# wizyoung/YOLOv3_TensorFlow

Measured on AMD Instinct MI355X. Metric: images/sec at 416x416 bs=32 (Darknet-53 + 3-scale head forward), higher is better.
Workload: dtype f32

## Files before the change

include/yolo355.h:

```cpp
#ifndef YOLO355_H
#define YOLO355_H

#include <stddef.h>
#include <stdint.h>

#ifdef __cplusplus
extern "C" {
#endif

#define Y3_OK 0
#define Y3_EINVAL (-1)
#define Y3_EHIP (-2)
#define Y3_ESTATE (-3)

#define Y3_ABI_VERSION 5

typedef struct y3_ctx y3_ctx;
typedef struct y3_net y3_net;
typedef struct y3_train_var y3_train_var;

const char* y3_last_error(void);
int y3_abi_version(void);

int y3_ctx_create(int device, void* stream, y3_ctx** out);
// ... 15 lines not shown
    int stride;
    int act;
} y3_conv_desc;

size_t y3_conv_workspace_bytes(const y3_conv_desc* d);
int y3_streamk_range(int kind, int units, int ksteps, int workers, int group, int local_worker, long long* begin,
                     long long* end);
int y3_conv_image_ranges(const y3_conv_desc* d, int dz_stride, long long limit, int max_ranges, int* begin, int* count);
void y3_debug_conv_range_limit(long long elements);
int y3_conv2d_fwd(y3_ctx* ctx, const y3_conv_desc* d, const float* x, const float* x_up,
                  const float* w, const float* scale, const float* shift, const float* residual,
                  float* y, void* workspace, size_t workspace_bytes);

int y3_conv2d_fwd_stem_s2(y3_ctx* ctx, int n, int h, int w, const float* x, const float* w0_hwio, const float* scale0,
                          const float* shift0, const float* w1_packed, const float* scale1, const float* shift1, float* y);

int y3_pack_conv_weights_bf16(y3_ctx* ctx, const float* w_hwio, int k, int cin, int cout, void* w_packed);
int y3_conv_bf16_tile(const y3_conv_desc* d);
int y3_conv2d_fwd_bf16(y3_ctx* ctx, const y3_conv_desc* d, const void* x, const void* x_up, const void* w,
                       const float* scale, const float* shift, const void* residual, void* y, int out_f32);

int y3_conv2d_fwd_bf16_stem_s2(y3_ctx* ctx, int n, int h, int w, const float* x, const float* w0_hwio, const float* scale0,
                               const float* shift0, const void* w1_packed, const float* scale1, const float* shift1, void* y);

int y3_resblock64_fwd_bf16(y3_ctx* ctx, int n, int h, int w, const void* x, const void* w2_packed, const float* scale2,
                           const float* shift2, const void* w3_packed, const float* scale3, const float* shift3, void* y);

int y3_conv_wino_eligible(const y3_conv_desc* d);
int y3_pack_conv_weights_wino(y3_ctx* ctx, const float* w_hwio, int cin, int cout, float* w_wino);
size_t y3_conv_wino_workspace_bytes(const y3_conv_desc* d);
// ... 40 lines not shown

int y3_net_create(y3_ctx* ctx, int class_num, y3_net** out);
int y3_net_destroy(y3_net* net);
int y3_net_set_dtype(y3_net* net, int dtype);
int y3_net_num_layers(const y3_net* net);
int y3_net_layer_info(const y3_net* net, int i, int* k, int* stride, int* cin, int* cout, int* has_bn);
size_t y3_net_params_bytes(const y3_net* net);
int y3_net_set_params(y3_net* net, const y3_train_var* vars, void* params, size_t params_bytes);
size_t y3_net_workspace_bytes(const y3_net* net, int n, int h, int w);
int y3_net_forward(y3_net* net, const float* x, int n, int h, int w, void* workspace,
                   size_t workspace_bytes, float* fm1, float* fm2, float* fm3);
int y3_net_set_profiling(y3_net* net, int enabled);
int y3_net_get_layer_ms(y3_net* net, float* ms, int count);
int y3_net_layer_is_streamk(const y3_net* net, int i, int n, int h, int w);
int y3_net_layer_fused(const y3_net* net, int i, int n, int h, int w);

int y3_net_layer_graph(const y3_net* net, int i, int* src, int* up, int* resid, int* dst, int* act);
int y3_net_num_tensors(const y3_net* net);
int y3_net_tensor_info(const y3_net* net, int t, int* channels, int* sdiv, int* ext);


size_t y3_reduce_scratch_bytes(int c);
int y3_bn_train_stats(y3_ctx* ctx, const float* z, long long rows, int c, const float* gamma, const float* beta,
                      float eps, float decay, float* mean, float* inv_std, float* scale, float* shift,
                      float* moving_mean, float* moving_var, float* scratch);
int y3_conv_stats_blocks(const y3_conv_desc* d, int wino);
int y3_conv2d_fwd_stats(y3_ctx* ctx, const y3_conv_desc* d, const float* x, const float* w, const float* scale,
                        const float* shift, float* y, float* stats, void* workspace, size_t workspace_bytes);
int y3_conv2d_fwd_wino_stats(y3_ctx* ctx, const y3_conv_desc* d, const float* x, const float* w_wino, const float* scale,
                             const float* shift, float* y, float* stats, void* workspace, size_t workspace_bytes);
// ... 197 lines not shown
```

yolov3_tensorflow_amd/_lib.py:

```python
import ctypes
import os
from ctypes import POINTER, c_char_p, c_double, c_float, c_int, c_longlong, c_size_t, c_void_p

HERE = os.path.dirname(os.path.abspath(__file__))
LIB_PATH = os.environ.get("Y3_LIB_PATH") or os.path.join(HERE, "csrc", "libyolo355.so")

Y3_OK, Y3_EINVAL, Y3_EHIP, Y3_ESTATE = 0, -1, -2, -3
Y3_NMS_TF, Y3_NMS_PY = 0, 1


class ConvDesc(ctypes.Structure):
    _fields_ = [(n, c_int) for n in ("n", "h", "w", "cin", "c_up", "cout", "k", "stride", "act")]


class ParamDesc(ctypes.Structure):
    _fields_ = [("w", c_void_p), ("g", c_void_p), ("slot0", c_void_p), ("slot1", c_void_p), ("n", c_longlong),
                ("weight_decay", c_float), ("reserved", c_int)]


class TrainVar(ctypes.Structure):
    _fields_ = [("weights", c_void_p), ("gamma", c_void_p), ("beta", c_void_p), ("moving_mean", c_void_p),
                ("moving_variance", c_void_p), ("biases", c_void_p), ("g_weights", c_longlong), ("g_gamma", c_longlong),
                ("g_beta", c_longlong), ("g_biases", c_longlong), ("g_end", c_longlong)]

# ... 42 lines not shown
                                   c_void_p, c_void_p, c_size_t]),
    "y3_pack_conv_weights_split": (c_int, [c_void_p, c_void_p, c_int, c_int, c_int, c_int, c_void_p]),
    "y3_conv2d_fwd_split": (c_int, [c_void_p, POINTER(ConvDesc), c_int, c_void_p, c_void_p, c_void_p, c_void_p,
                                    c_void_p, c_void_p, c_void_p, c_void_p, c_size_t]),
    "y3_pack_conv_weights_split_dgrad": (c_int, [c_void_p, c_void_p, c_int, c_int, c_int, c_int, c_void_p]),
    "y3_conv2d_dgrad_split": (c_int, [c_void_p, POINTER(ConvDesc), c_int, c_void_p, c_int, c_void_p, c_void_p, c_void_p,
                                      c_int, c_void_p, c_void_p, c_size_t]),
    "y3_pack_conv_weights_bf16": (c_int, [c_void_p, c_void_p, c_int, c_int, c_int, c_void_p]),
    "y3_conv_bf16_tile": (c_int, [POINTER(ConvDesc)]),
    "y3_conv2d_fwd_bf16": (c_int, [c_void_p, POINTER(ConvDesc), c_void_p, c_void_p, c_void_p, c_void_p, c_void_p,
                                   c_void_p, c_void_p, c_int]),
    "y3_conv2d_fwd_bf16_stem_s2": (c_int, [c_void_p, c_int, c_int, c_int, c_void_p, c_void_p, c_void_p, c_void_p, c_void_p,
                                           c_void_p, c_void_p, c_void_p]),
    "y3_conv2d_fwd_stem_s2": (c_int, [c_void_p, c_int, c_int, c_int, c_void_p, c_void_p, c_void_p, c_void_p, c_void_p,
                                      c_void_p, c_void_p, c_void_p]),
    "y3_resblock64_fwd_bf16": (c_int, [c_void_p, c_int, c_int, c_int, c_void_p, c_void_p, c_void_p, c_void_p, c_void_p,
                                       c_void_p, c_void_p, c_void_p]),
    "y3_net_train_workspace_bytes": (c_size_t, [c_void_p, POINTER(TrainVar), c_int, c_int, c_int]),
    "y3_net_train_forward": (c_int, [c_void_p, POINTER(TrainVar), c_void_p, c_int, c_int, c_int, POINTER(TrainOpts),
                                     c_void_p, c_size_t, POINTER(c_void_p), POINTER(c_void_p), POINTER(c_void_p)]),
    "y3_net_train_loss": (c_int, [c_void_p, c_void_p, c_void_p, c_void_p, POINTER(TrainOpts), c_void_p]),
    "y3_net_train_backward": (c_int, [c_void_p, POINTER(TrainVar), c_void_p, GradReadyFn, c_void_p]),
    "y3_net_train_step": (c_int, [c_void_p, POINTER(TrainVar), c_void_p, c_int, c_int, c_int, c_void_p, c_void_p, c_void_p,
                                  POINTER(TrainOpts), c_void_p, c_void_p, c_size_t, c_void_p, GradReadyFn, c_void_p]),
    "y3_net_train_set_wgrad_stream": (c_int, [c_void_p, c_void_p]),
    "y3_net_train_set_box_loss": (c_int, [c_void_p, c_int]),
    "y3_net_train_set_bn_sync": (c_int, [c_void_p, BnSyncFn, c_void_p, c_void_p, c_size_t]),
    "y3_net_train_saved": (c_int, [c_void_p, c_int, POINTER(c_size_t), POINTER(c_size_t)]),
    "y3_net_train_saved_type": (c_int, [c_void_p, c_int]),
    "y3_pack_conv_weights_bf16_train": (c_int, [c_void_p, c_void_p, c_int, c_int, c_int, c_int, c_void_p]),
# ... 158 lines not shown
```

yolov3_tensorflow_amd/csrc/y3_abi.hip:

```cpp
#include <cstdarg>
#include <cstdio>
#include <cstring>
#include <vector>
#include <algorithm>
#include "y3_internal.h"
#include "y3_net.h"

static thread_local char g_err[512] = "";

void y3_set_error(const char* fmt, ...) {
    va_list ap;
    va_start(ap, fmt);
    vsnprintf(g_err, sizeof(g_err), fmt, ap);
    va_end(ap);
}

extern "C" const char* y3_last_error(void) { return g_err; }

int y3_current_device() {
    int dev = -1;
    if (hipGetDevice(&dev) != hipSuccess || dev < 0 || dev >= Y3_MAX_DEVICES) return -1;
    return dev;
}

// ... 364 lines not shown

extern "C" int y3_net_set_dtype(y3_net* net, int dtype) {
    Y3_CHECK_ARG(net, "y3_net_set_dtype: null net");
    Y3_CHECK_ARG(dtype >= 0 && dtype <= 4,
                 "y3_net_set_dtype: dtype must be 0 (fp32), 1 (bf16), 2 (fp32 via bf16x6), 3 (fp32 via bf16x3) or "
                 "4 (fp32, Winograd for the eligible 3x3 convs)");
    net->dtype = static_cast<NetDtype>(dtype);
    net->pn = net->ph = net->pw = 0;
    for (Layer& l : net->layers) {
        l.scale = l.shift = nullptr;
        std::fill(std::begin(l.w), std::end(l.w), nullptr);
    }
    return Y3_OK;
}

extern "C" int y3_net_destroy(y3_net* net) {
    if (net) {
        for (auto& set : net->event_sets)
            for (hipEvent_t e : set) (void)hipEventDestroy(e);
        if (net->train) y3_train_state_free(net->train);
        if (net->own_stream) (void)hipStreamDestroy(static_cast<hipStream_t>(net->own_stream));
        delete net;
    }
    return Y3_OK;
}

extern "C" int y3_net_num_layers(const y3_net* net) { return net ? (int)net->layers.size() : 0; }

extern "C" int y3_net_layer_info(const y3_net* net, int i, int* k, int* stride, int* cin, int* cout,
                                 int* has_bn) {
// ... 43 lines not shown

static bool fuses_with_next(const y3_net& net, int j, int n, int h, int w) {
    const NetDtype dt = net.dtype;
    const Layer &a = net.layers[j], &b = net.layers[j + 1];
    const Tensor &mid = net.tensors[a.dst], &out = net.tensors[b.dst];
    const y3_conv_desc da = net.desc(j, n, h, w), db = net.desc(j + 1, n, h, w);
    const bool pair = b.src == a.dst && mid.last_use == j + 1 && mid.ext < 0 && out.ext < 0 && a.resid < 0;
    if (j == 0)
        return pair && a.src == 0 && b.resid < 0 &&
               (dt == NetDtype::BF16 ? y3_conv_bf16_stem_s2_takes(&da, &db)
                : (dt == NetDtype::F32 || dt == NetDtype::F32_WINO) && y3_conv_f32_stem_s2_takes(&da, &db)) == 1;
    return j == 2 && dt == NetDtype::BF16 && pair && b.resid == a.src && a.src != 0 && net.tensors[a.src].ext < 0 &&
           y3_conv_bf16_resblock64_takes(&da, &db) == 1;
}

static int split_planes(NetDtype dt) { return dt == NetDtype::F32_BF16X6 ? 3 : dt == NetDtype::F32_BF16X3 ? 2 : 0; }

static ConvRoute fp32_route(const y3_conv_desc& d, bool wino44, bool wino, int planes) {
    ConvRoute r;
    r.kind = wino44 ? RouteKind::Wino44 : wino ? RouteKind::Wino : planes ? RouteKind::Split : RouteKind::Direct;
    r.planes = planes;
    r.two_pass = wino44 && y3_conv_wino44_two_pass_impl(&d);
    r.streamk = !wino44 && !wino && y3_conv_schedule_impl(&d);
    r.scratch = wino44 ? (r.two_pass ? y3_conv_wino44_workspace_bytes_impl(&d) : 0)
                : wino ? y3_conv_wino_workspace_bytes_impl(&d) : y3_conv_workspace_bytes_impl(&d);
    return r;
}

ConvRoute y3_route_infer(const y3_net& net, int i, int n, int h, int w) {
    ConvRoute r;
    const NetDtype dt = net.dtype;
    const y3_conv_desc d = net.desc(i, n, h, w);
    if ((i == 0 || i == 2) && fuses_with_next(net, i, n, h, w)) r.kind = RouteKind::InNext;
    else if ((i == 1 || i == 3) && fuses_with_next(net, i - 1, n, h, w))
        r.kind = i == 3 ? RouteKind::ResBlock64Bf16 : dt == NetDtype::BF16 ? RouteKind::StemS2Bf16 : RouteKind::StemS2F32;
    else if (dt == NetDtype::BF16) r.kind = RouteKind::Bf16;
    else
        r = fp32_route(d, dt == NetDtype::F32_WINO && y3_conv_wino44_preferred_impl(&d),
                       dt == NetDtype::F32_WINO && y3_conv_wino_eligible_impl(&d), split_planes(dt));
    return r;
}

static bool bf16_train(const y3_net& net, int i) { return net.dtype == NetDtype::BF16 && net.layers[i].cin != 3; }

ConvRoute y3_route_train_fwd(const y3_net& net, int i, int n, int h, int w) {
    const Layer& l = net.layers[i];
    const y3_conv_desc d = net.desc(i, n, h, w, true);
    if (bf16_train(net, i)) {
        ConvRoute r;
        r.kind = RouteKind::Bf16Train;
// ... 44 lines not shown
    return r;
}

ConvPack y3_conv_pack(const y3_net& net, int i, const ConvRoute& r, bool dgrad) {
    const Layer& l = net.layers[i];
    ConvPack p;
    p.planes = r.planes; p.dgrad = dgrad;
    p.k = l.k; p.cin = l.cin; p.cout = dgrad ? net.dz_stride(i) : l.cout;
    p.wcout = l.cout;
    switch (r.kind) {
    case RouteKind::Wino44: p.kind = Packing::Wino44; break;
    case RouteKind::Wino: p.kind = Packing::Wino; break;
    case RouteKind::Split: p.kind = Packing::Split; break;
    case RouteKind::Bf16: case RouteKind::StemS2Bf16: case RouteKind::ResBlock64Bf16: p.kind = Packing::Bf16; break;
    case RouteKind::InNext: p.kind = net.dtype == NetDtype::BF16 ? Packing::Bf16 : Packing::Direct; break;
    case RouteKind::Direct: case RouteKind::StemS2F32: p.kind = dgrad ? Packing::Hwio : Packing::Direct; break;
    case RouteKind::Bf16Train: p.kind = Packing::Bf16Reg; break;
    }
    if (l.cin == 3 && !dgrad) p.kind = Packing::Hwio;
    return p;
}

size_t ConvPack::bytes() const {
    const size_t taps = (size_t)k * k * cin * cout;
    switch (kind) {
    case Packing::Direct: return taps * 4;
    case Packing::Bf16: case Packing::Bf16Reg: return taps * 2;
    case Packing::Split: return taps * 2 * planes;
    case Packing::Wino: return (size_t)16 * cin * cout * 4;
    case Packing::Wino44: return (size_t)36 * cin * cout * 4;
    default: return 0;
// ... 90 lines not shown
        }
    }
    for (size_t i = 0; i < net->layers.size(); ++i) {
        Layer& l = net->layers[i];
        l.scale = reinterpret_cast<const float*>(base + lp[i].scale);
        l.shift = reinterpret_cast<const float*>(base + lp[i].shift);
        std::fill(std::begin(l.w), std::end(l.w), nullptr);
        for (size_t j = 0; j < lp[i].packs.size(); ++j) l.w[(int)lp[i].packs[j].kind] = base + lp[i].at[j];
    }
    return Y3_OK;
}

extern "C" int y3_net_layer_fused(const y3_net* net, int i, int n, int h, int w) {
    if (!net || i < 0 || i >= (int)net->layers.size() || n <= 0 || h <= 0 || w <= 0) return 0;
    const RouteKind k = y3_route_infer(*net, i, n, h, w).kind;
    return k == RouteKind::InNext ? 1 : k >= RouteKind::StemS2F32 ? 2 : 0;
}

extern "C" int y3_net_forward(y3_net* net, const float* x, int n, int h, int w, void* workspace,
                              size_t workspace_bytes, float* fm1, float* fm2, float* fm3) {
    Y3_CHECK_ARG(net && x && workspace && fm1 && fm2 && fm3, "y3_net_forward: null argument");
    if (!net->ctx) {
        y3_set_error("y3_net_forward: the net was created without a context");
        return Y3_ESTATE;
    }
    if (int rc = ctx_pending_error(net->ctx)) return rc;
    if (int rc = check_size("y3_net_forward", n, h, w)) return rc;
    net->plan(n, h, w);
    Y3_CHECK_ARG(workspace_bytes >= net->plan_bytes, "y3_net_forward: workspace too small (%zu < %zu)",
                 workspace_bytes, net->plan_bytes);
    Y3_CHECK_ARG(((uintptr_t)workspace & 255) == 0, "y3_net_forward: workspace must be 256-byte aligned");
// ... 30 lines not shown
    if (net->flags_bytes) Y3_CHECK_HIP(hipMemsetAsync(flag_base, 0, net->flags_bytes, st));
    void* scratch = base + net->arena_bytes; const size_t sb = net->scratch_bytes;
    for (size_t i = 0; i < nl; ++i) {
        const Layer& l = net->layers[i];
        const ConvRoute& r = net->routes[i];
        const y3_conv_desc d = net->desc((int)i, n, h, w);
        y3_sk_opts o;
        o.err = net->ctx->err_host;
        o.flags = net->flags_bytes ? flag_base + i * y3_net::FLAG_WORDS : nullptr;
        o.wino44_form = r.two_pass;
        const Layer& p = net->layers[i ? i - 1 : 0];
        const float *pw = wk[i ? i - 1 : 0], *lw = wk[i];
        float *src = ptr(l.src), *up = ptr(l.up), *res = ptr(l.resid), *y = ptr(l.dst);
        int rc = Y3_OK;
        switch (r.kind) {
        case RouteKind::InNext: break;
        case RouteKind::StemS2F32:
            rc = y3_launch_conv_f32_stem_s2(st, n, h, w, x, pw, p.scale, p.shift, p.act, lw, l.scale, l.shift, l.act, y); break;
        case RouteKind::StemS2Bf16:
            rc = y3_launch_conv_bf16_stem_s2(st, n, h, w, x, pw, p.scale, p.shift, p.act, lw, l.scale, l.shift, l.act, y); break;
        case RouteKind::ResBlock64Bf16:
            rc = y3_launch_conv_bf16_resblock64(st, n, d.h, d.w, ptr(p.src), pw, p.scale, p.shift, p.act, lw, l.scale, l.shift,
                                                l.act, y);
            break;
        case RouteKind::Bf16:
            rc = y3_launch_conv_bf16(st, &d, src, up, lw, l.scale, l.shift, res, y, net->tensors[l.dst].ext >= 0 ? 1 : 0); break;
        case RouteKind::Wino44: rc = y3_launch_conv_wino44(st, &d, src, lw, l.scale, l.shift, res, y, scratch, sb, &o); break;
        case RouteKind::Wino: rc = y3_launch_conv_wino(st, &d, src, lw, l.scale, l.shift, res, y, scratch, sb, &o); break;
        case RouteKind::Split:
            rc = y3_launch_conv_split(st, &d, r.planes, src, up, lw, l.scale, l.shift, res, y, scratch, sb, &o); break;
        case RouteKind::Direct: rc = y3_launch_conv(st, &d, src, up, lw, l.scale, l.shift, res, y, scratch, sb, &o); break;
        case RouteKind::Bf16Train: y3_set_error("y3_net_forward: layer %d has a train-step route", i); return Y3_EINVAL;
        }
// ... 40 lines not shown
```

yolov3_tensorflow_amd/csrc/y3_conv_f32s.hip:

```cpp
#include <cstdlib>
#include "y3_lds.h"

namespace {

struct StemS2F32Args {
    const float* x;
    const float* w0;
    const float* scale0;
    const float* shift0;
    const float* w1;
    const float* scale1;
    const float* shift1;
    float* y;
    int N, H, W, act0, act1;
    int tiles_y, tiles_x, ntiles;
};

constexpr int TSY = 8, TSX = 16;
constexpr int SPY = 2 * TSY + 1, SPX = 2 * TSX + 1;
constexpr int NSP = SPY * SPX;
constexpr int PPY = SPY + 2, PPX = SPX + 2;
constexpr int PATCH_FLOATS = PPY * PPX * 3;
constexpr int SIDX = TSX + 1;
constexpr int S_BYTES = 2 * SPY * SIDX * 128;
constexpr int W1_BYTES = 9 * 64 * 128;
constexpr int P_BYTES = ((PATCH_FLOATS + 1) * 4 + 15) & ~15;
constexpr int LDS_BYTES = S_BYTES + W1_BYTES + P_BYTES;
constexpr int NTHR = 512, NW = 8;
constexpr int NPRE = (PPY * PPX + NTHR - 1) / NTHR;
constexpr int OPITCH = 144;

__global__ void __launch_bounds__(NTHR) conv_stem_s2_f32_kernel(const StemS2F32Args p) {
    extern __shared__ __attribute__((aligned(16))) unsigned char smem[];
    unsigned char* S = smem;
    unsigned char* W1 = smem + S_BYTES;
    float* P = reinterpret_cast<float*>(smem + S_BYTES + W1_BYTES);

    const int tid = threadIdx.x, lane = tid & 63;
    const int wave = __builtin_amdgcn_readfirstlane(tid >> 6);
    const int l32 = lane & 31, h = lane >> 5;
    const int OH = p.H >> 1, OW = p.W >> 1;

    for (int c = tid; c < 9 * 64 * 8; c += NTHR) {
        const int row = c >> 3, ch = c & 7;
        const u32x4 v = *reinterpret_cast<const u32x4*>(p.w1 + (size_t)row * 32 + ch * 4);
        *reinterpret_cast<u32x4*>(W1 + row * 128 + ((ch ^ ((row >> 1) & 7)) << 4)) = v;
// ... 7 lines not shown
    }
    int koff[14];
#pragma unroll
    for (int j = 0; j < 14; ++j) {
        const int k = 2 * j + h;
        koff[j] = k < 27 ? (k + 96 * (k / 9)) * 4 : -1;
    }
    const int rt = wave >> 2, ct = wave & 3;
    f32x4 sc0[4], sh0[4], sc1[4], sh1[4];
#pragma unroll
    for (int g = 0; g < 4; ++g) {
        sc0[g] = *reinterpret_cast<const f32x4*>(p.scale0 + 8 * g + 4 * h);
        sh0[g] = *reinterpret_cast<const f32x4*>(p.shift0 + 8 * g + 4 * h);
        sc1[g] = *reinterpret_cast<const f32x4*>(p.scale1 + 32 * rt + 8 * g + 4 * h);
        sh1[g] = *reinterpret_cast<const f32x4*>(p.shift1 + 32 * rt + 8 * g + 4 * h);
    }

    const int G = gridDim.x;
    int tile = blockIdx.x;
    float pre[NPRE][3];
    int prow[NPRE], pcol[NPRE];
#pragma unroll
    for (int j = 0; j < NPRE; ++j) {
        const int e = tid + NTHR * j;
        prow[j] = e < PPY * PPX ? e / PPX : -1000000;
        pcol[j] = e - (e / PPX) * PPX;
    }
    auto prefetch = [&](int t) {
        const int tpi = p.tiles_y * p.tiles_x;
        const int n = t / tpi, r = t - n * tpi;
// ... 72 lines not shown
            const unsigned char* ap = W1 + row * 128;
            const int asw = (row >> 1) & 7;
            const int idx = oxl + (kx >> 1);
            const unsigned char* bp = S + (((kx & 1) * SPY + 2 * oyl + ky) * SIDX + idx) * 128;
            const int bsw = (idx >> 1) & 7;
#pragma unroll
            for (int kk = 0; kk < 4; ++kk) {
                const f32x4 a = *reinterpret_cast<const f32x4*>(ap + (((2 * kk + h) ^ asw) << 4));
                const f32x4 b = *reinterpret_cast<const f32x4*>(bp + (((2 * kk + h) ^ bsw) << 4));
#pragma unroll
                for (int q = 0; q < 4; ++q) acc3 = __builtin_amdgcn_mfma_f32_32x32x2f32(a[q], b[q], acc3, 0, 0, 0);
            }
        }
        __syncthreads();
        unsigned char* out = S + wave * (32 * OPITCH);
#pragma unroll
        for (int g = 0; g < 4; ++g) {
            f32x4 o;
#pragma unroll
            for (int e = 0; e < 4; ++e) {
                const float t = acc3[4 * g + e] * sc1[g][e] + sh1[g][e];
                o[e] = p.act1 ? fmaxf(t, 0.1f * t) : t;
            }
            *reinterpret_cast<f32x4*>(out + l32 * OPITCH + (8 * g + 4 * h) * 4) = o;
        }
#pragma unroll
        for (int i = 0; i < 4; ++i) {
            const int pl = i * 8 + (lane >> 3), piece = lane & 7;
            const int mm = ct * 32 + pl;
            const int oy = oy0 + (mm >> 4), ox = ox0 + (mm & 15);
            const f32x4 v = *reinterpret_cast<const f32x4*>(out + pl * OPITCH + piece * 16);
            if (oy < OH && ox < OW)
                *reinterpret_cast<f32x4*>(p.y + ((size_t)(n * OH + oy) * OW + ox) * 64 + rt * 32 + piece * 4) = v;
        }
        __syncthreads();
    }
}

}

int y3_conv_f32_stem_s2_takes(const y3_conv_desc* d0, const y3_conv_desc* d1) {
    if (!d0 || !d1) return 0;
    static int off = -1;
    if (off < 0) {
        const char* e = y3_exp_env("Y3_F32_FUSED_STEM");
        off = (e && e[0] == '0') ? 1 : 0;
    }
    if (off) return 0;
    if (y3_device_max_lds() < (size_t)LDS_BYTES) return 0;
    return d0->k == 3 && d0->stride == 1 && d0->cin == 3 && d0->cout == 32 && d0->c_up == 0 &&
           d1->k == 3 && d1->stride == 2 && d1->cin == 32 && d1->cout == 64 && d1->c_up == 0 &&
           d1->n == d0->n && d1->h == d0->h && d1->w == d0->w && d0->h % 2 == 0 && d0->w % 2 == 0;
}

int y3_launch_conv_f32_stem_s2(hipStream_t stream, int n, int h, int w, const float* x, const float* w0, const float* scale0,
                               const float* shift0, int act0, const float* w1_packed, const float* scale1, const float* shift1,
                               int act1, float* y) {
    Y3_CHECK_ARG(x && w0 && scale0 && shift0 && w1_packed && scale1 && shift1 && y, "y3_conv2d_fwd_stem_s2: null pointer argument");
    Y3_CHECK_ARG(n > 0 && h > 0 && w > 0 && h % 2 == 0 && w % 2 == 0, "y3_conv2d_fwd_stem_s2: the image sides must be even");
    Y3_CHECK_ARG((long long)n * h * w * 16 < (1LL << 31), "y3_conv2d_fwd_stem_s2: tensor too large for 32-bit pixel indices");
    StemS2F32Args a;
    a.x = x; a.w0 = w0; a.scale0 = scale0; a.shift0 = shift0; a.w1 = w1_packed; a.scale1 = scale1; a.shift1 = shift1; a.y = y;
    a.N = n; a.H = h; a.W = w; a.act0 = act0; a.act1 = act1;
    a.tiles_y = (h / 2 + TSY - 1) / TSY; a.tiles_x = (w / 2 + TSX - 1) / TSX;
    a.ntiles = n * a.tiles_y * a.tiles_x;
    const int grid = a.ntiles < 256 ? a.ntiles : 256;
    return y3_launch_lds<conv_stem_s2_f32_kernel>(stream, dim3(grid), dim3(NTHR), LDS_BYTES, a);
}

extern "C" int y3_conv2d_fwd_stem_s2(y3_ctx* ctx, int n, int h, int w, const float* x, const float* w0_hwio, const float* scale0,
                                     const float* shift0, const float* w1_packed, const float* scale1, const float* shift1,
                                     float* y) {
    Y3_CHECK_ARG(ctx, "y3_conv2d_fwd_stem_s2: null context");
    return y3_launch_conv_f32_stem_s2(ctx->stream, n, h, w, x, w0_hwio, scale0, shift0, 1, w1_packed, scale1, shift1, 1, y);
}
```

yolov3_tensorflow_amd/csrc/y3_internal.h:

```cpp
#pragma once
#include <hip/hip_runtime.h>
#include <stdint.h>
#include <stddef.h>
#include "../../include/yolo355.h"

struct y3_ctx {
    int device;
    hipStream_t stream;
    unsigned* err_host;
    void* stage_host = nullptr;
    size_t stage_bytes = 0;
    hipEvent_t stage_ev = nullptr;
    bool stage_busy = false;
};
int y3_ctx_stage_acquire(y3_ctx* ctx, size_t bytes, void** out);
int y3_ctx_stage_release(y3_ctx* ctx);
int ctx_pending_error(const y3_ctx* ctx);

struct y3_sk_opts {
    unsigned* flags = nullptr;
    unsigned* err = nullptr;
    float* stats = nullptr;
    const float* bwd_z = nullptr;
    const float* bwd_vec = nullptr;
// ... 82 lines not shown
                        const float* scale, const float* shift, const void* residual, void* y, int out_f32);
int y3_conv_bf16_train_stats_blocks(const y3_conv_desc* d);
int y3_launch_conv_bf16_train(hipStream_t stream, const y3_conv_desc* d, const void* x, const void* w, void* z, float* stats);
int y3_launch_conv_bf16_reg(hipStream_t stream, const y3_conv_desc* d, const void* x, const void* w, const float* scale,
                            const float* shift, void* y, int out_f32);
int y3_launch_conv_bf16_dgrad(hipStream_t stream, const y3_conv_desc* fwd, const void* dz, int dz_stride, const void* w_d,
                              int accumulate, float* dx);
int y3_pack_conv_weights_bf16_reg(y3_ctx* ctx, const float* w_hwio, int k, int cin, int cout, int dgrad_stride, void* w_packed);
int y3_launch_conv_wgrad_bf16(hipStream_t stream, const y3_conv_desc* d, const void* x, const void* dz, int dz_stride, float* dw,
                              void* scratch, size_t scratch_bytes);
int y3_conv_bf16x_takes(int k, int cin);
int y3_launch_pack_bf16x(hipStream_t stream, const float* w_hwio, int k, int cin, int cout, void* w_packed);
int y3_launch_conv_bf16x(hipStream_t stream, const y3_conv_desc* d, const void* x, const void* x_up, const void* w,
                         const float* scale, const float* shift, const void* residual, void* y, int out_f32);
int y3_conv_f32_stem_s2_takes(const y3_conv_desc* d0, const y3_conv_desc* d1);
int y3_launch_conv_f32_stem_s2(hipStream_t stream, int n, int h, int w, const float* x, const float* w0, const float* scale0,
                               const float* shift0, int act0, const float* w1_packed, const float* scale1, const float* shift1,
                               int act1, float* y);
int y3_conv_bf16_stem_s2_takes(const y3_conv_desc* d0, const y3_conv_desc* d1);
int y3_launch_conv_bf16_stem_s2(hipStream_t stream, int n, int h, int w, const float* x, const float* w0, const float* scale0,
                                const float* shift0, int act0, const void* w1_packed, const float* scale1, const float* shift1,
                                int act1, void* y);
int y3_conv_bf16_resblock64_takes(const y3_conv_desc* d2, const y3_conv_desc* d3);
int y3_launch_conv_bf16_resblock64(hipStream_t stream, int n, int h, int w, const void* x, const void* w2_packed,
                                   const float* scale2, const float* shift2, int act2, const void* w3_packed, const float* scale3,
                                   const float* shift3, int act3, void* y);
int y3_conv_bf16r_takes(int k, int cin);
int y3_conv_bf16r_tile(const y3_conv_desc* d);
int y3_launch_conv_bf16r(hipStream_t stream, const y3_conv_desc* d, const void* x, const void* x_up, const void* w,
                         const float* scale, const float* shift, const void* residual, void* y, int out_f32);
int y3_launch_pack_split(hipStream_t stream, const float* w_hwio, int k, int cin, int cout, int planes, void* out,
                         int transposed = 0);
int y3_launch_conv_dgrad_split(hipStream_t stream, const y3_conv_desc* fwd, int planes, const float* dz, int dz_stride,
// ... 28 lines not shown
```

yolov3_tensorflow_amd/csrc/y3_net.h:

```cpp
#pragma once
#include <vector>
#include <algorithm>
#include "y3_internal.h"

enum class NetDtype { F32 = 0, BF16 = 1, F32_BF16X6 = 2, F32_BF16X3 = 3, F32_WINO = 4 };

enum class RouteKind { Direct, Split, Wino, Wino44, Bf16, InNext, StemS2F32, StemS2Bf16, ResBlock64Bf16, Bf16Train };
struct ConvRoute {
    RouteKind kind = RouteKind::Direct;
    int planes = 0;
    bool two_pass = false;
    bool streamk = false;
    size_t scratch = 0;
    int bn_blocks = 0;
};
struct y3_net;
ConvRoute y3_route_infer(const y3_net& net, int i, int n, int h, int w);
ConvRoute y3_route_train_fwd(const y3_net& net, int i, int n, int h, int w);
ConvRoute y3_route_dgrad(const y3_net& net, int i, int n, int h, int w);
ConvRoute y3_route_wgrad(const y3_net& net, int i, int n, int h, int w);

enum class Packing { Hwio, Direct, Bf16, Split, Wino, Wino44, Bf16Reg, Count };
struct ConvPack {
    Packing kind = Packing::Hwio;
    int planes = 0;
    bool dgrad = false;
    int k = 0, cin = 0, cout = 0;
// ... 74 lines not shown

struct y3_train_state;
void y3_train_state_free(y3_train_state* s);

struct y3_net {
    y3_ctx* ctx;
    int class_num;
    y3_train_state* train = nullptr;
    void* wgrad_stream = nullptr;
    int box_loss = Y3_BOX_MSE;
    void* own_stream = nullptr;
    y3_bn_sync_fn bn_sync_fn = nullptr;
    void* bn_sync_user = nullptr;
    double* bn_sync_buf = nullptr;
    NetDtype dtype = NetDtype::F32;
    std::vector<Tensor> tensors;
    std::vector<Layer> layers;
    int pn = 0, ph = 0, pw = 0;
    std::vector<size_t> offsets;
    size_t plan_bytes = 0;
    size_t arena_bytes = 0;
    size_t scratch_bytes = 0;
    std::vector<ConvRoute> routes;
    size_t flags_bytes = 0;
    static constexpr size_t FLAG_WORDS = 512;
    bool profiling = false;
    std::vector<std::vector<hipEvent_t>> event_sets;
    size_t sets_used = 0;

    int add_conv(int src, int cout, int k, int stride = 1, bool bn = true, bool act = true, int resid = -1,
// ... 107 lines not shown
```

yolov3_tensorflow_amd/model.py:

```python
from __future__ import division, print_function

import ctypes

import numpy as np
import torch

from . import _lib
from . import engine
from . import framework as fw
from .utils.layer_utils import conv2d, darknet53_body, yolo_block, upsample_layer, _conv_layer

N_BODY_CONVS = 52
NET_DTYPES = {'f32': 0, 'bf16': 1, 'f32_bf16x6': 2, 'f32_bf16x3': 3, 'f32_wino': 4}


BOX_LOSSES = {'mse': 0, 'giou': 1, 'diou': 2, 'ciou': 3}


_SIDE_STREAMS = {}

class yolov3(object):

    def __init__(self, class_num, anchors, use_label_smooth=False, use_focal_loss=False,
                 batch_norm_decay=0.999, weight_decay=5e-4, use_static_shape=True):
# ... 50 lines not shown
        return layers

    def _get_net(self, device):
        if self.compute_dtype not in NET_DTYPES:
            raise ValueError("compute_dtype must be one of %s" % (sorted(NET_DTYPES),))
        ctx = fw.context(device)
        scope = fw.current_scope_name()
        key = (ctx.value, scope, self.compute_dtype)
        ent = self._nets.get(key)
        L = _lib.lib()
        if ent is None:
            h = ctypes.c_void_p()
            _lib.check(L.y3_net_create(ctx, int(self.class_num), ctypes.byref(h)))
            if NET_DTYPES[self.compute_dtype]:
                _lib.check(L.y3_net_set_dtype(h, NET_DTYPES[self.compute_dtype]))
            table = self._layer_table(h)
            ent = dict(handle=h, table=table, params=None, ws=None, ws_bytes=0,
                       layers=self._ensure_variables(scope, table))
            self._nets[key] = ent
        pkey = (str(device), scope, self.compute_dtype)
        p = self._params.get(pkey)
        if p is None or p['checked'] != fw.global_version():
            versions = tuple(v.version for layer in ent['layers'] for v in
                             ((layer[0],) + tuple(layer[1] or ()) + ((layer[2],) if layer[2] is not None else ())))
            if p is None or p['versions'] != versions:
                if p is None:
                    nbytes = L.y3_net_params_bytes(ent['handle'])
                    p = dict(buf=torch.empty(nbytes, dtype=torch.uint8, device=device), bytes=nbytes)
                    self._params[pkey] = p
                from . import training
# ... 112 lines not shown
        ent = self._get_net(device if device is not None else fw.default_device())
        _lib.check(_lib.lib().y3_net_set_profiling(ent['handle'], 1 if enabled else 0))
        self._profiling_on = bool(enabled)

    def read_layer_ms(self, device=None):
        ent = self._get_net(device if device is not None else fw.default_device())
        nl = len(ent['table'])
        buf = (ctypes.c_float * nl)()
        _lib.check(_lib.lib().y3_net_get_layer_ms(ent['handle'], buf, nl))
        return np.array(buf[:], dtype=np.float64), ent['table']

    def layer_is_streamk(self, n, h, w, device=None):
        ent = self._get_net(device if device is not None else fw.default_device())
        L = _lib.lib()
        return np.array([L.y3_net_layer_is_streamk(ent['handle'], i, n, h, w) for i in range(len(ent['table']))], bool)

    def layer_fused(self, n, h, w, device=None):
        ent = self._get_net(device if device is not None else fw.default_device())
        L = _lib.lib()
        return np.array([L.y3_net_layer_fused(ent['handle'], i, n, h, w) for i in range(len(ent['table']))], int)

    def layer_times_ms(self, inputs, iters=5):
        x = fw.as_device_f32(inputs)
        self.forward(x)
        self.set_layer_profiling(True, x.device)
        for _ in range(iters):
            self.forward(x)
        ms, table = self.read_layer_ms(x.device)
        self.set_layer_profiling(False, x.device)
        return ms, table
# ... 67 lines not shown
```

Measured before the change: 3355.

## Fuse the first 1x1 pointwise conv into the f32 stride-2 stem kernel epilogue

```diff
diff --git a/include/yolo355.h b/include/yolo355.h
--- a/include/yolo355.h
+++ b/include/yolo355.h
@@ -53,6 +53,9 @@
 
 int y3_conv2d_fwd_stem_s2(y3_ctx* ctx, int n, int h, int w, const float* x, const float* w0_hwio, const float* scale0,
                           const float* shift0, const float* w1_packed, const float* scale1, const float* shift1, float* y);
+int y3_conv2d_fwd_stem_s2_pw(y3_ctx* ctx, int n, int h, int w, const float* x, const float* w0_hwio, const float* scale0,
+                             const float* shift0, const float* w1_packed, const float* scale1, const float* shift1, float* y,
+                             const float* w2_packed, const float* scale2, const float* shift2, float* y2);
 
 int y3_pack_conv_weights_bf16(y3_ctx* ctx, const float* w_hwio, int k, int cin, int cout, void* w_packed);
 int y3_conv_bf16_tile(const y3_conv_desc* d);
@@ -123,6 +126,8 @@
 int y3_net_get_layer_ms(y3_net* net, float* ms, int count);
 int y3_net_layer_is_streamk(const y3_net* net, int i, int n, int h, int w);
 int y3_net_layer_fused(const y3_net* net, int i, int n, int h, int w);
+int y3_net_layer_is_tail(const y3_net* net, int i, int n, int h, int w);
+int y3_net_set_pointwise_fusion(y3_net* net, int enabled);
 
 int y3_net_layer_graph(const y3_net* net, int i, int* src, int* up, int* resid, int* dst, int* act);
 int y3_net_num_tensors(const y3_net* net);
diff --git a/yolov3_tensorflow_amd/_lib.py b/yolov3_tensorflow_amd/_lib.py
--- a/yolov3_tensorflow_amd/_lib.py
+++ b/yolov3_tensorflow_amd/_lib.py
@@ -80,6 +80,10 @@
                                            c_void_p, c_void_p, c_void_p]),
     "y3_conv2d_fwd_stem_s2": (c_int, [c_void_p, c_int, c_int, c_int, c_void_p, c_void_p, c_void_p, c_void_p, c_void_p,
                                       c_void_p, c_void_p, c_void_p]),
+    "y3_conv2d_fwd_stem_s2_pw": (c_int, [c_void_p, c_int, c_int, c_int, c_void_p, c_void_p, c_void_p, c_void_p, c_void_p,
+                                         c_void_p, c_void_p, c_void_p, c_void_p, c_void_p, c_void_p, c_void_p]),
+    "y3_net_set_pointwise_fusion": (c_int, [c_void_p, c_int]),
+    "y3_net_layer_is_tail": (c_int, [c_void_p, c_int, c_int, c_int, c_int]),
     "y3_resblock64_fwd_bf16": (c_int, [c_void_p, c_int, c_int, c_int, c_void_p, c_void_p, c_void_p, c_void_p, c_void_p,
                                        c_void_p, c_void_p, c_void_p]),
     "y3_net_train_workspace_bytes": (c_size_t, [c_void_p, POINTER(TrainVar), c_int, c_int, c_int]),
diff --git a/yolov3_tensorflow_amd/csrc/y3_abi.hip b/yolov3_tensorflow_amd/csrc/y3_abi.hip
--- a/yolov3_tensorflow_amd/csrc/y3_abi.hip
+++ b/yolov3_tensorflow_amd/csrc/y3_abi.hip
@@ -402,6 +402,13 @@
     return Y3_OK;
 }
 
+extern "C" int y3_net_set_pointwise_fusion(y3_net* net, int enabled) {
+    Y3_CHECK_ARG(net, "y3_net_set_pointwise_fusion: null net");
+    net->pointwise_fusion = enabled != 0;
+    net->pn = net->ph = net->pw = 0;
+    return Y3_OK;
+}
+
 extern "C" int y3_net_destroy(y3_net* net) {
     if (net) {
         for (auto& set : net->event_sets)
@@ -475,6 +482,16 @@
            y3_conv_bf16_resblock64_takes(&da, &db) == 1;
 }
 
+static bool runs_next_as_tail(const y3_net& net, int j, int n, int h, int w) {
+    const NetDtype dt = net.dtype;
+    if (!net.pointwise_fusion || j < 0 || j + 1 >= (int)net.layers.size() || (dt != NetDtype::F32 && dt != NetDtype::F32_WINO)) return false;
+    const Layer &a = net.layers[j], &b = net.layers[j + 1];
+    if (!(b.k == 1 && b.stride == 1 && b.resid < 0 && b.up < 0 && b.src == a.dst)) return false;
+    const y3_conv_desc da = net.desc(j, n, h, w), db = net.desc(j + 1, n, h, w);
+    if (j == 1 && fuses_with_next(net, 0, n, h, w)) return y3_conv_f32_stem_s2_tail_takes(&da, &db) == 1;
+    return false;
+}
+
 static int split_planes(NetDtype dt) { return dt == NetDtype::F32_BF16X6 ? 3 : dt == NetDtype::F32_BF16X3 ? 2 : 0; }
 
 static ConvRoute fp32_route(const y3_conv_desc& d, bool wino44, bool wino, int planes) {
@@ -492,9 +509,12 @@
     ConvRoute r;
     const NetDtype dt = net.dtype;
     const y3_conv_desc d = net.desc(i, n, h, w);
-    if ((i == 0 || i == 2) && fuses_with_next(net, i, n, h, w)) r.kind = RouteKind::InNext;
-    else if ((i == 1 || i == 3) && fuses_with_next(net, i - 1, n, h, w))
+    if (runs_next_as_tail(net, i - 1, n, h, w)) r.kind = RouteKind::InPrev;
+    else if ((i == 0 || i == 2) && fuses_with_next(net, i, n, h, w)) r.kind = RouteKind::InNext;
+    else if ((i == 1 || i == 3) && fuses_with_next(net, i - 1, n, h, w)) {
         r.kind = i == 3 ? RouteKind::ResBlock64Bf16 : dt == NetDtype::BF16 ? RouteKind::StemS2Bf16 : RouteKind::StemS2F32;
+        r.tail = runs_next_as_tail(net, i, n, h, w);
+    }
     else if (dt == NetDtype::BF16) r.kind = RouteKind::Bf16;
     else
         r = fp32_route(d, dt == NetDtype::F32_WINO && y3_conv_wino44_preferred_impl(&d),
@@ -569,7 +589,7 @@
     case RouteKind::Split: p.kind = Packing::Split; break;
     case RouteKind::Bf16: case RouteKind::StemS2Bf16: case RouteKind::ResBlock64Bf16: p.kind = Packing::Bf16; break;
     case RouteKind::InNext: p.kind = net.dtype == NetDtype::BF16 ? Packing::Bf16 : Packing::Direct; break;
-    case RouteKind::Direct: case RouteKind::StemS2F32: p.kind = dgrad ? Packing::Hwio : Packing::Direct; break;
+    case RouteKind::Direct: case RouteKind::StemS2F32: case RouteKind::InPrev: p.kind = dgrad ? Packing::Hwio : Packing::Direct; break;
     case RouteKind::Bf16Train: p.kind = Packing::Bf16Reg; break;
     }
     if (l.cin == 3 && !dgrad) p.kind = Packing::Hwio;
@@ -690,7 +710,12 @@
 extern "C" int y3_net_layer_fused(const y3_net* net, int i, int n, int h, int w) {
     if (!net || i < 0 || i >= (int)net->layers.size() || n <= 0 || h <= 0 || w <= 0) return 0;
     const RouteKind k = y3_route_infer(*net, i, n, h, w).kind;
-    return k == RouteKind::InNext ? 1 : k >= RouteKind::StemS2F32 ? 2 : 0;
+    return k == RouteKind::InNext ? 1 : k == RouteKind::InPrev ? 0 : k >= RouteKind::StemS2F32 ? 2 : 0;
+}
+
+extern "C" int y3_net_layer_is_tail(const y3_net* net, int i, int n, int h, int w) {
+    if (!net || i < 0 || i >= (int)net->layers.size() || n <= 0 || h <= 0 || w <= 0) return 0;
+    return y3_route_infer(*net, i, n, h, w).kind == RouteKind::InPrev;
 }
 
 extern "C" int y3_net_forward(y3_net* net, const float* x, int n, int h, int w, void* workspace,
@@ -751,9 +776,14 @@
         float *src = ptr(l.src), *up = ptr(l.up), *res = ptr(l.resid), *y = ptr(l.dst);
         int rc = Y3_OK;
         switch (r.kind) {
-        case RouteKind::InNext: break;
-        case RouteKind::StemS2F32:
-            rc = y3_launch_conv_f32_stem_s2(st, n, h, w, x, pw, p.scale, p.shift, p.act, lw, l.scale, l.shift, l.act, y); break;
+        case RouteKind::InNext: case RouteKind::InPrev: break;
+        case RouteKind::StemS2F32: {
+            const Layer& t = net->layers[r.tail ? i + 1 : i];
+            const y3_pw_tail tail = {wk[r.tail ? i + 1 : i], t.scale, t.shift, t.act, ptr(t.dst)};
+            rc = y3_launch_conv_f32_stem_s2(st, n, h, w, x, pw, p.scale, p.shift, p.act, lw, l.scale, l.shift, l.act, y,
+                                            r.tail ? &tail : nullptr);
+            break;
+        }
         case RouteKind::StemS2Bf16:
             rc = y3_launch_conv_bf16_stem_s2(st, n, h, w, x, pw, p.scale, p.shift, p.act, lw, l.scale, l.shift, l.act, y); break;
         case RouteKind::ResBlock64Bf16:
diff --git a/yolov3_tensorflow_amd/csrc/y3_conv_f32s.hip b/yolov3_tensorflow_amd/csrc/y3_conv_f32s.hip
--- a/yolov3_tensorflow_amd/csrc/y3_conv_f32s.hip
+++ b/yolov3_tensorflow_amd/csrc/y3_conv_f32s.hip
@@ -14,6 +14,11 @@
     float* y;
     int N, H, W, act0, act1;
     int tiles_y, tiles_x, ntiles;
+    int act2;
+    const float* w2;
+    const float* scale2;
+    const float* shift2;
+    float* y2;
 };
 
 constexpr int TSY = 8, TSX = 16;
@@ -29,7 +34,11 @@
 constexpr int NTHR = 512, NW = 8;
 constexpr int NPRE = (PPY * PPX + NTHR - 1) / NTHR;
 constexpr int OPITCH = 144;
-
+constexpr int STAGE_BYTES = NW * 32 * OPITCH;
+constexpr int XCH_BYTES = 4 * 16 * 64 * 4;
+static_assert(STAGE_BYTES + XCH_BYTES <= S_BYTES, "the epilogue's staging must fit the idle stem-pixel LDS");
+
+template <bool PW>
 __global__ void __launch_bounds__(NTHR) conv_stem_s2_f32_kernel(const StemS2F32Args p) {
     extern __shared__ __attribute__((aligned(16))) unsigned char smem[];
     unsigned char* S = smem;
@@ -67,6 +76,15 @@
         sh0[g] = *reinterpret_cast<const f32x4*>(p.shift0 + 8 * g + 4 * h);
         sc1[g] = *reinterpret_cast<const f32x4*>(p.scale1 + 32 * rt + 8 * g + 4 * h);
         sh1[g] = *reinterpret_cast<const f32x4*>(p.shift1 + 32 * rt + 8 * g + 4 * h);
+    }
+    f32x4 w2r[PW ? 4 : 1], sc2[PW ? 4 : 1], sh2[PW ? 4 : 1];
+    if (PW) {
+#pragma unroll
+        for (int g = 0; g < 4; ++g) {
+            w2r[PW ? g : 0] = *reinterpret_cast<const f32x4*>(p.w2 + l32 * 64 + 32 * rt + 8 * g + 4 * h);
+            sc2[PW ? g : 0] = *reinterpret_cast<const f32x4*>(p.scale2 + 8 * g + 4 * h);
+            sh2[PW ? g : 0] = *reinterpret_cast<const f32x4*>(p.shift2 + 8 * g + 4 * h);
+        }
     }
 
     const int G = gridDim.x;
@@ -169,24 +187,85 @@
         }
         __syncthreads();
         unsigned char* out = S + wave * (32 * OPITCH);
-#pragma unroll
-        for (int g = 0; g < 4; ++g) {
-            f32x4 o;
-#pragma unroll
-            for (int e = 0; e < 4; ++e) {
-                const float t = acc3[4 * g + e] * sc1[g][e] + sh1[g][e];
-                o[e] = p.act1 ? fmaxf(t, 0.1f * t) : t;
-            }
-            *reinterpret_cast<f32x4*>(out + l32 * OPITCH + (8 * g + 4 * h) * 4) = o;
-        }
-#pragma unroll
-        for (int i = 0; i < 4; ++i) {
-            const int pl = i * 8 + (lane >> 3), piece = lane & 7;
-            const int mm = ct * 32 + pl;
-            const int oy = oy0 + (mm >> 4), ox = ox0 + (mm & 15);
-            const f32x4 v = *reinterpret_cast<const f32x4*>(out + pl * OPITCH + piece * 16);
-            if (oy < OH && ox < OW)
-                *reinterpret_cast<f32x4*>(p.y + ((size_t)(n * OH + oy) * OW + ox) * 64 + rt * 32 + piece * 4) = v;
+        auto stage_store = [&](const f32x4 (&v)[4], float* dst, int cstride, int coff) {
+#pragma unroll
+            for (int g = 0; g < 4; ++g) *reinterpret_cast<f32x4*>(out + l32 * OPITCH + (8 * g + 4 * h) * 4) = v[g];
+#pragma unroll
+            for (int i = 0; i < 4; ++i) {
+                const int pl = i * 8 + (lane >> 3), piece = lane & 7;
+                const int mm = ct * 32 + pl;
+                const int oy = oy0 + (mm >> 4), ox = ox0 + (mm & 15);
+                const f32x4 v4 = *reinterpret_cast<const f32x4*>(out + pl * OPITCH + piece * 16);
+                if (oy < OH && ox < OW)
+                    *reinterpret_cast<f32x4*>(dst + ((size_t)(n * OH + oy) * OW + ox) * cstride + coff + piece * 4) = v4;
+            }
+        };
+        if (!PW) {
+#pragma unroll
+            for (int g = 0; g < 4; ++g) {
+                f32x4 o;
+#pragma unroll
+                for (int e = 0; e < 4; ++e) {
+                    const float t = acc3[4 * g + e] * sc1[g][e] + sh1[g][e];
+                    o[e] = p.act1 ? fmaxf(t, 0.1f * t) : t;
+                }
+                *reinterpret_cast<f32x4*>(out + l32 * OPITCH + (8 * g + 4 * h) * 4) = o;
+            }
+#pragma unroll
+            for (int i = 0; i < 4; ++i) {
+                const int pl = i * 8 + (lane >> 3), piece = lane & 7;
+                const int mm = ct * 32 + pl;
+                const int oy = oy0 + (mm >> 4), ox = ox0 + (mm & 15);
+                const f32x4 v = *reinterpret_cast<const f32x4*>(out + pl * OPITCH + piece * 16);
+                if (oy < OH && ox < OW)
+                    *reinterpret_cast<f32x4*>(p.y + ((size_t)(n * OH + oy) * OW + ox) * 64 + rt * 32 + piece * 4) = v;
+            }
+        } else {
+            f32x4 o[4];
+#pragma unroll
+            for (int g = 0; g < 4; ++g)
+#pragma unroll
+                for (int e = 0; e < 4; ++e) {
+                    const float t = acc3[4 * g + e] * sc1[g][e] + sh1[g][e];
+                    o[g][e] = p.act1 ? fmaxf(t, 0.1f * t) : t;
+                }
+            __builtin_amdgcn_s_waitcnt(0x0F70);
+            float* xch = reinterpret_cast<float*>(S + STAGE_BYTES) + ct * (16 * 64);
+            f32x16 acc5;
+            if (rt == 0) {
+#pragma unroll
+                for (int q = 0; q < 16; ++q) acc5[q] = 0.f;
+#pragma unroll
+                for (int g = 0; g < 4; ++g)
+#pragma unroll
+                    for (int e = 0; e < 4; ++e)
+                        acc5 = __builtin_amdgcn_mfma_f32_32x32x2f32(w2r[PW ? g : 0][e], o[g][e], acc5, 0, 0, 0);
+#pragma unroll
+                for (int q = 0; q < 16; ++q) xch[q * 64 + lane] = acc5[q];
+            } else {
+                stage_store(o, p.y, 64, 32);
+            }
+            __syncthreads();
+            if (rt == 0) {
+                stage_store(o, p.y, 64, 0);
+            } else {
+#pragma unroll
+                for (int q = 0; q < 16; ++q) acc5[q] = xch[q * 64 + lane];
+#pragma unroll
+                for (int g = 0; g < 4; ++g)
+#pragma unroll
+                    for (int e = 0; e < 4; ++e)
+                        acc5 = __builtin_amdgcn_mfma_f32_32x32x2f32(w2r[PW ? g : 0][e], o[g][e], acc5, 0, 0, 0);
+                f32x4 o2[4];
+#pragma unroll
+                for (int g = 0; g < 4; ++g)
+#pragma unroll
+                    for (int e = 0; e < 4; ++e) {
+                        const float t = acc5[4 * g + e] * sc2[PW ? g : 0][e] + sh2[PW ? g : 0][e];
+                        o2[g][e] = p.act2 ? fmaxf(t, 0.1f * t) : t;
+                    }
+                stage_store(o2, p.y2, 32, 0);
+            }
         }
         __syncthreads();
     }
@@ -208,24 +287,42 @@
            d1->n == d0->n && d1->h == d0->h && d1->w == d0->w && d0->h % 2 == 0 && d0->w % 2 == 0;
 }
 
+int y3_conv_f32_stem_s2_tail_takes(const y3_conv_desc* d1, const y3_conv_desc* d2) {
+    if (!d1 || !d2) return 0;
+    return d2->k == 1 && d2->stride == 1 && d2->cin == 64 && d2->cout == 32 && d2->c_up == 0 && d1->cout == 64 && d1->stride == 2 &&
+           d2->n == d1->n && d2->h == d1->h / 2 && d2->w == d1->w / 2;
+}
+
 int y3_launch_conv_f32_stem_s2(hipStream_t stream, int n, int h, int w, const float* x, const float* w0, const float* scale0,
                                const float* shift0, int act0, const float* w1_packed, const float* scale1, const float* shift1,
-                               int act1, float* y) {
+                               int act1, float* y, const y3_pw_tail* tail) {
     Y3_CHECK_ARG(x && w0 && scale0 && shift0 && w1_packed && scale1 && shift1 && y, "y3_conv2d_fwd_stem_s2: null pointer argument");
+    Y3_CHECK_ARG(!tail || (tail->w && tail->scale && tail->shift && tail->y), "y3_conv2d_fwd_stem_s2_pw: null pointer argument");
     Y3_CHECK_ARG(n > 0 && h > 0 && w > 0 && h % 2 == 0 && w % 2 == 0, "y3_conv2d_fwd_stem_s2: the image sides must be even");
     Y3_CHECK_ARG((long long)n * h * w * 16 < (1LL << 31), "y3_conv2d_fwd_stem_s2: tensor too large for 32-bit pixel indices");
     StemS2F32Args a;
     a.x = x; a.w0 = w0; a.scale0 = scale0; a.shift0 = shift0; a.w1 = w1_packed; a.scale1 = scale1; a.shift1 = shift1; a.y = y;
+    a.w2 = tail ? tail->w : nullptr; a.scale2 = tail ? tail->scale : nullptr; a.shift2 = tail ? tail->shift : nullptr;
+    a.y2 = tail ? tail->y : nullptr; a.act2 = tail ? tail->act : 0;
     a.N = n; a.H = h; a.W = w; a.act0 = act0; a.act1 = act1;
     a.tiles_y = (h / 2 + TSY - 1) / TSY; a.tiles_x = (w / 2 + TSX - 1) / TSX;
     a.ntiles = n * a.tiles_y * a.tiles_x;
     const int grid = a.ntiles < 256 ? a.ntiles : 256;
-    return y3_launch_lds<conv_stem_s2_f32_kernel>(stream, dim3(grid), dim3(NTHR), LDS_BYTES, a);
+    if (tail) return y3_launch_lds<conv_stem_s2_f32_kernel<true>>(stream, dim3(grid), dim3(NTHR), LDS_BYTES, a);
+    return y3_launch_lds<conv_stem_s2_f32_kernel<false>>(stream, dim3(grid), dim3(NTHR), LDS_BYTES, a);
 }
 
 extern "C" int y3_conv2d_fwd_stem_s2(y3_ctx* ctx, int n, int h, int w, const float* x, const float* w0_hwio, const float* scale0,
                                      const float* shift0, const float* w1_packed, const float* scale1, const float* shift1,
                                      float* y) {
     Y3_CHECK_ARG(ctx, "y3_conv2d_fwd_stem_s2: null context");
-    return y3_launch_conv_f32_stem_s2(ctx->stream, n, h, w, x, w0_hwio, scale0, shift0, 1, w1_packed, scale1, shift1, 1, y);
-}
+    return y3_launch_conv_f32_stem_s2(ctx->stream, n, h, w, x, w0_hwio, scale0, shift0, 1, w1_packed, scale1, shift1, 1, y, nullptr);
+}
+
+extern "C" int y3_conv2d_fwd_stem_s2_pw(y3_ctx* ctx, int n, int h, int w, const float* x, const float* w0_hwio, const float* scale0,
+                                        const float* shift0, const float* w1_packed, const float* scale1, const float* shift1,
+                                        float* y, const float* w2_packed, const float* scale2, const float* shift2, float* y2) {
+    Y3_CHECK_ARG(ctx, "y3_conv2d_fwd_stem_s2_pw: null context");
+    const y3_pw_tail tail = {w2_packed, scale2, shift2, 1, y2};
+    return y3_launch_conv_f32_stem_s2(ctx->stream, n, h, w, x, w0_hwio, scale0, shift0, 1, w1_packed, scale1, shift1, 1, y, &tail);
+}
diff --git a/yolov3_tensorflow_amd/csrc/y3_internal.h b/yolov3_tensorflow_amd/csrc/y3_internal.h
--- a/yolov3_tensorflow_amd/csrc/y3_internal.h
+++ b/yolov3_tensorflow_amd/csrc/y3_internal.h
@@ -120,9 +120,15 @@
 int y3_launch_conv_bf16x(hipStream_t stream, const y3_conv_desc* d, const void* x, const void* x_up, const void* w,
                          const float* scale, const float* shift, const void* residual, void* y, int out_f32);
 int y3_conv_f32_stem_s2_takes(const y3_conv_desc* d0, const y3_conv_desc* d1);
+struct y3_pw_tail {
+    const float *w, *scale, *shift;
+    int act;
+    float* y;
+};
+int y3_conv_f32_stem_s2_tail_takes(const y3_conv_desc* d1, const y3_conv_desc* d2);
 int y3_launch_conv_f32_stem_s2(hipStream_t stream, int n, int h, int w, const float* x, const float* w0, const float* scale0,
                                const float* shift0, int act0, const float* w1_packed, const float* scale1, const float* shift1,
-                               int act1, float* y);
+                               int act1, float* y, const y3_pw_tail* tail = nullptr);
 int y3_conv_bf16_stem_s2_takes(const y3_conv_desc* d0, const y3_conv_desc* d1);
 int y3_launch_conv_bf16_stem_s2(hipStream_t stream, int n, int h, int w, const float* x, const float* w0, const float* scale0,
                                 const float* shift0, int act0, const void* w1_packed, const float* scale1, const float* shift1,
diff --git a/yolov3_tensorflow_amd/csrc/y3_net.h b/yolov3_tensorflow_amd/csrc/y3_net.h
--- a/yolov3_tensorflow_amd/csrc/y3_net.h
+++ b/yolov3_tensorflow_amd/csrc/y3_net.h
@@ -5,12 +5,13 @@
 
 enum class NetDtype { F32 = 0, BF16 = 1, F32_BF16X6 = 2, F32_BF16X3 = 3, F32_WINO = 4 };
 
-enum class RouteKind { Direct, Split, Wino, Wino44, Bf16, InNext, StemS2F32, StemS2Bf16, ResBlock64Bf16, Bf16Train };
+enum class RouteKind { Direct, Split, Wino, Wino44, Bf16, InNext, StemS2F32, StemS2Bf16, ResBlock64Bf16, InPrev, Bf16Train };
 struct ConvRoute {
     RouteKind kind = RouteKind::Direct;
     int planes = 0;
     bool two_pass = false;
     bool streamk = false;
+    bool tail = false;
     size_t scratch = 0;
     int bn_blocks = 0;
 };
@@ -115,6 +116,7 @@
     void* bn_sync_user = nullptr;
     double* bn_sync_buf = nullptr;
     NetDtype dtype = NetDtype::F32;
+    bool pointwise_fusion = true;
     std::vector<Tensor> tensors;
     std::vector<Layer> layers;
     int pn = 0, ph = 0, pw = 0;
diff --git a/yolov3_tensorflow_amd/model.py b/yolov3_tensorflow_amd/model.py
--- a/yolov3_tensorflow_amd/model.py
+++ b/yolov3_tensorflow_amd/model.py
@@ -88,6 +88,8 @@
             _lib.check(L.y3_net_create(ctx, int(self.class_num), ctypes.byref(h)))
             if NET_DTYPES[self.compute_dtype]:
                 _lib.check(L.y3_net_set_dtype(h, NET_DTYPES[self.compute_dtype]))
+            if not getattr(self, '_pointwise_fusion', True):
+                _lib.check(L.y3_net_set_pointwise_fusion(h, 0))
             table = self._layer_table(h)
             ent = dict(handle=h, table=table, params=None, ws=None, ws_bytes=0,
                        layers=self._ensure_variables(scope, table))
@@ -230,6 +232,16 @@
         ent = self._get_net(device if device is not None else fw.default_device())
         L = _lib.lib()
         return np.array([L.y3_net_layer_is_streamk(ent['handle'], i, n, h, w) for i in range(len(ent['table']))], bool)
+
+    def set_pointwise_fusion(self, enabled):
+        self._pointwise_fusion = bool(enabled)
+        for ent in self._nets.values():
+            _lib.check(_lib.lib().y3_net_set_pointwise_fusion(ent['handle'], 1 if enabled else 0))
+
+    def layer_is_tail(self, n, h, w, device=None):
+        ent = self._get_net(device if device is not None else fw.default_device())
+        L = _lib.lib()
+        return np.array([L.y3_net_layer_is_tail(ent['handle'], i, n, h, w) for i in range(len(ent['table']))], bool)
 
     def layer_fused(self, n, h, w, device=None):
         ent = self._get_net(device if device is not None else fw.default_device())
```

Result: no change. 3372, median of 6 (+0.5%).
